# 236088/reflect-sampling-nerf

Hardware: AMD Instinct MI355X
Metric: rays/sec (train step) at 4096 rays x 128 samples, 1/2/4/8 MI355X; PSNR vs ref (higher is better)
Workload: dtype f32

## Files before the change

### reflect_sampling_nerf_amd/csrc/rsn_common.h

```cpp
#pragma once
#include <hip/hip_runtime.h>
#include <stdint.h>
#include <stdio.h>

#include "rsn.h"

#define RSN_K_ENC_PAD 104
#define RSN_K_SH_PAD 40
#define RSN_ENC_ITS (RSN_K_ENC_PAD / 8)
#define RSN_SH_ITS (RSN_K_SH_PAD / 8)
#define RSN_ENC_K16 7
#define RSN_SH_K16 3
#define RSN_AUX_ITS 6

void rsn_set_error(const char* fmt, ...);
int rsn_device_cus();

#define RSN_REQUIRE(cond, code, ...)        \
  do {                                      \
    if (!(cond)) {                          \
      rsn_set_error(__VA_ARGS__);           \
      return (code);                        \
    }                                       \
  } while (0)

#define RSN_TRY(call)                       \
  do {                                      \
    const int rc_ = (call);                 \
    if (rc_ != RSN_OK) return rc_;          \
  } while (0)

#define RSN_HIP(call)                                                                   \
  do {                                                                                  \
    hipError_t e_ = (call);                                                             \
    if (e_ != hipSuccess) {                                                             \
      rsn_set_error("%s failed: %s (%s:%d)", #call, hipGetErrorString(e_), __FILE__, __LINE__); \
      return RSN_ERR_HIP;                                                               \
    }                                                                                   \
  } while (0)

struct RsnPackedLayout {
  int nb;
  int nbm;
  size_t w_x[RSN_MAX_TRUNK_LAYERS];
  size_t w_enc0;
  size_t w_enc_skip;
  size_t b[RSN_MAX_TRUNK_LAYERS];
  size_t w_bh, b_bh;
  size_t w_mid_sh, w_mid_x, b_mid;
  size_t w_rgb, b_rgb;
  size_t wT_x[RSN_MAX_TRUNK_LAYERS];
  size_t wT_enc0, wT_enc_skip;
  size_t wT_bh;
  size_t wT_mid_x;
  size_t wT_rgb;
  size_t v_density;
  size_t h_x[RSN_MAX_TRUNK_LAYERS];
  size_t h_enc0, h_enc_skip, h_bh, h_mid_sh, h_mid_x, h_rgb;
  size_t hT_x[RSN_MAX_TRUNK_LAYERS];
  size_t hT_enc0, hT_enc_skip, hT_bh, hT_mid_x, hT_rgb;
  size_t hT_seed;
  size_t q_stream;
  int q_groups;
  int t_g_begin, t_g_trunk, t_g_encskip, t_g_enc0, t_g_end;
  int q_pf;
  size_t fold_wc, fold_bc, w_fold, b_fold, wT_fold;
  size_t total;
};
#define RSN_RING_GROUP_FRAGS 16
#define RSN_RING_MAX_LAYERS 10
inline bool rsn_ring_training(const rsn_field_desc* d) {
  return (d->mma_mode == RSN_MMA_BF16 || d->mma_mode == RSN_MMA_BF16X6) && d->width == 256 &&
         d->num_layers <= RSN_RING_MAX_LAYERS;
}

int rsn_compute_layout(const rsn_field_desc* desc, RsnPackedLayout* L);

__device__ __forceinline__ float rsn_seed_product(float w, float wd) { return w * wd; }
```

### reflect_sampling_nerf_amd/csrc/rsn_field_bwd.hip

```cpp
#include "rsn_mfma.h"

#include "rsn_field_common.h"
#include "rsn_field_bwd_common.h"

template <int NB, int MMA>
__global__ __launch_bounds__(256) void rsn_field_bwd_kernel(const BwdJobs J) {
  constexpr bool FOLD = MMA == RSN_MMA_F32_FOLDED;
  constexpr int MODE = FOLD ? 0 : MMA;
  constexpr int HIT = FOLD ? 16 : NB * 4;
  constexpr int XITS = (NB * 4 > 16) ? NB * 4 : 16;
  constexpr int WAVE_F4 = (XITS + RSN_AUX_ITS) * 64;
  constexpr int W = NB * 32;
  constexpr bool SBF = MODE == 3;
  __shared__ float4 smem[4 * WAVE_F4];

  const int lane = threadIdx.x & 63;
  const int wid = __builtin_amdgcn_readfirstlane(threadIdx.x >> 6);
  float4* X = smem + wid * WAVE_F4 + lane;
  float* Xf = reinterpret_cast<float*>(X);

  const BwdShared& P = J.s;
  const TileJobs T = tile_space<128>(J);
  const float* __restrict__ pk = P.packed;
  const float4 zero4 = make_float4(0.0f, 0.0f, 0.0f, 0.0f);

  for (long long gtile = blockIdx.x; gtile < T.n_tiles; gtile += gridDim.x) {
    const TileAt ta = tile_at(T, gtile);
    const BwdJob& a = J.j[ta.job];
    const long long n_points = ta.n_points, tile = ta.tile;
    const long long p0 = tile * 128 + wid * 32;
    if (p0 >= n_points) continue;
    int ln = lane;
    asm volatile("" : "+v"(ln));
    const int m = ln & 31, h = ln >> 5;
    const long long p = p0 + m;
    const bool valid = p < n_points;
    const long long pc = valid ? p : n_points - 1;
    const int rows = (int)(n_points - p0 < 32 ? n_points - p0 : 32);
    constexpr bool LOOPST = MODE == 0;
    auto rb_epi = [&](float* base, long long elem, int row_elems) {
      return rowbuf<SBF>(LOOPST ? nullptr : base, elem, rows, row_elems, m, h);
    };
    auto rb_loop = [&](float* base, long long elem, int row_elems) {
      return rowbuf<false>(LOOPST ? base : nullptr, elem, rows, row_elems, m, h);
    };
    const float live = valid ? 1.0f : 0.0f;

    auto bits_at = [&](int l) -> const unsigned* {
      return a.saved.relu_bits + ((((long long)l * (a.act_stride / W)) + pc) * 2 + h) * (NB / 2 > 2 ? NB / 2 : 2);
    };
    HeadGradIn hg;
    head_grad_inputs(a, pc, live, h == 1 && valid, hg);

    X[0] = (h == 1) ? make_float4(hg.dz[0], hg.dz[1], hg.dz[2], 0.0f) : zero4;
    X[64] = zero4; X[128] = zero4; X[192] = zero4;
    {
      const ReluBits<4> mb = load_relu_bits<4>(bits_at(P.num_layers));
      __builtin_amdgcn_sched_barrier(0);
      f32x16 acc[4];
      zero_acc<4>(acc);
      gemm_mode<MODE, 4, 4, true>(acc, pk + P.L.wT_rgb, pk + P.L.hT_rgb, X, 4, ln);
      store_masked_bits<4, SBF>(acc, X, mb, h, rb_epi(a.gout.da_mid, p0 * 128, 128));
    }
    if constexpr (!FOLD) {
      f32x16 acc[NB];
      zero_acc<NB>(acc);
      gemm_mode<MODE, NB, NB, true>(acc, pk + P.L.wT_mid_x, pk + P.L.hT_mid_x, X, 16, ln, rb_loop(a.gout.da_mid, p0 * 128, 128));
      store_act<NB, NB, false, SBF>(acc, X, rb_epi(a.gout.d_bott, p0 * W, W), h);
    }
    {
      const float4 q0 = head_grad_row<false>(h == 0 ? 0 : 1, a, P.density_bias, pc, live, hg);
      const float4 q1 = head_grad_row<false>(h == 0 ? 2 : 3, a, P.density_bias, pc, live, hg);
      X[(HIT + 0) * 64] = q0;
      X[(HIT + 1) * 64] = q1;
      X[(HIT + 2) * 64] = zero4;
      X[(HIT + 3) * 64] = zero4;
      if (valid && a.gout.dz_heads) {
        *reinterpret_cast<float4*>(a.gout.dz_heads + pc * 16 + 4 * h) = q0;
        *reinterpret_cast<float4*>(a.gout.dz_heads + pc * 16 + 8 + 4 * h) = q1;
      }
      const int l = P.num_layers - 1;
      const ReluBits<NB> mb = load_relu_bits<NB>(bits_at(l));
      __builtin_amdgcn_sched_barrier(0);
      f32x16 acc[NB];
      zero_acc<NB>(acc);
      if constexpr (FOLD)
        gemm_mode<MODE, NB, NB, true>(acc, pk + P.L.wT_fold, pk + P.L.hT_bh, X, 16 + 4, ln, rb_loop(a.gout.da_mid, p0 * 128, 128));
      else
        gemm_mode<MODE, NB, NB, true>(acc, pk + P.L.wT_bh, pk + P.L.hT_bh, X, NB * 4 + 4, ln, rb_loop(a.gout.d_bott, p0 * W, W));
      store_masked_bits<NB, SBF>(acc, X, mb, h, rb_epi(a.gout.dy, (long long)l * a.act_stride + p0 * W, W));
    }
    f32x16 eacc[4];
    zero_acc<4>(eacc);
#pragma unroll 1
    for (int l = P.num_layers - 1; l >= 1; --l) {
      if (a.need_input_grad && l == P.skip_layer)
        gemm_mode<MODE, 4, 4, true>(eacc, pk + P.L.wT_enc_skip, pk + P.L.hT_enc_skip, X, NB * 4, ln);
      const ReluBits<NB> mb = load_relu_bits<NB>(bits_at(l - 1));
      __builtin_amdgcn_sched_barrier(0);
      f32x16 acc[NB];
      zero_acc<NB>(acc);
      gemm_mode<MODE, NB, NB, true>(acc, pk + P.L.wT_x[l], pk + P.L.hT_x[l], X, NB * 4, ln,
                          rb_loop(a.gout.dy, (long long)l * a.act_stride + p0 * W, W));
      store_masked_bits<NB, SBF>(acc, X, mb, h, rb_epi(a.gout.dy, (long long)(l - 1) * a.act_stride + p0 * W, W));
    }
    if (LOOPST && !a.need_input_grad) {
      const RowBuf r0 = rb_loop(a.gout.dy, p0 * W, W);
#pragma unroll 4
      for (int it = 0; it < NB * 4; ++it) sv_put_it(r0, it, X[it * 64]);
    }
    if (a.need_input_grad) {
      gemm_mode<MODE, 4, 4, true>(eacc, pk + P.L.wT_enc0, pk + P.L.hT_enc0, X, NB * 4, ln, rb_loop(a.gout.dy, p0 * W, W));
      store_act<4, 4, false>(eacc, X);
      const float* encp = a.saved.enc + pc * RSN_K_ENC_PAD;
      float dvar[3];
#pragma unroll 1
      for (int c = 0; c < 3; ++c) {
        float part = 0.0f;
#pragma unroll 2
        for (int jj = 0; jj < 8; ++jj) {
          const float f = h ? P.freqs[8 + jj] : P.freqs[jj];
          const int u = c * 8 + jj, u2 = u + 24;
          const float gs = Xf[(u >> 2) * 256 + (u & 3)], gc = Xf[(u2 >> 2) * 256 + (u2 & 3)];
          const float fs = encp[(u >> 2) * 8 + 4 * h + (u & 3)], fc = encp[(u2 >> 2) * 8 + 4 * h + (u2 & 3)];
          part += (-0.5f * (f * f)) * (gs * fs + gc * fc);
        }
        const float tot = part + __shfl_xor(part, 32, 64);
        if (c == 0) dvar[0] = tot; else if (c == 1) dvar[1] = tot; else dvar[2] = tot;
      }
      if (h == 0 && valid && a.gout.d_input) a.gout.d_input[pc] = input_grad_of_dvar(a, pc, dvar);
    }
  }
}

static int launch_bwd_jobs(const rsn_field_desc* d, const float* packed, BwdJob* js, int n, void* stream) {
  RSN_REQUIRE(n >= 1 && n <= RSN_MAX_JOBS, RSN_ERR_INVALID_ARGUMENT, "n_jobs=%d (1..%d)", n, RSN_MAX_JOBS);
  BwdJobs J = {};
  RSN_TRY(rsn_fill_shared(J.s, d, packed));
  for (int k = 0; k < n; ++k) {
    BwdJob& a = js[k];
    RSN_REQUIRE(a.saved.relu_bits && a.saved.heads && a.gout.dy, RSN_ERR_INVALID_ARGUMENT,
                "job %d: saved relu_bits / heads and gout.dy are required", k);
    RSN_REQUIRE(!a.need_input_grad || (a.saved.enc && a.gout.d_input), RSN_ERR_INVALID_ARGUMENT,
                "job %d: need_input_grad needs saved.enc and gout.d_input", k);
    RSN_REQUIRE(a.mode == RSN_MODE_INF || (a.fwd.raw_density && a.fwd.diff && a.fwd.tint), RSN_ERR_INVALID_ARGUMENT,
                "job %d: forward values raw_density/diff/tint are required", k);
    RSN_REQUIRE(!(a.gin.ray_pn_loss || a.gin.ray_ori_loss) || (a.mode == RSN_MODE_FRUSTUM && a.gin.weights),
                RSN_ERR_INVALID_ARGUMENT, "job %d: fused normal losses need the level's weights (frustum levels only)", k);
    RSN_REQUIRE(!a.gin.ray_pn_loss || (a.saved.normals && a.fwd.pred_normals), RSN_ERR_INVALID_ARGUMENT,
                "job %d: ray_pn_loss needs saved.normals and the forward pred_normals", k);
    RSN_REQUIRE(!a.gin.ray_ori_loss || a.fwd.n_dot_d, RSN_ERR_INVALID_ARGUMENT, "job %d: ray_ori_loss needs the forward n_dot_d", k);
    if (a.n_rays <= 0) continue;
    a.act_stride = (long long)a.n_rays * a.S * (long long)d->width;
    J.j[J.n_jobs++] = a;
  }
  if (J.n_jobs == 0) return RSN_OK;
  const long long n_tiles = rsn_job_tiles(J, 128);
  const int cached_cus = rsn_device_cus();
  const long long grid = n_tiles < (long long)cached_cus ? n_tiles : (long long)cached_cus;
  hipStream_t st = (hipStream_t)stream;
  const bool x6 = d->mma_mode == RSN_MMA_BF16X6;
  if (rsn_ring_training(d))
    return x6 ? rsn_launch_field_x6_bwd(n_tiles, st, J) : rsn_launch_field_bf16_bwd(rsn_job_tiles(J, 256), st, J);
#define RSN_LAUNCH_BWD(NBV)                                                                                  \
  do {                                                                                                       \
    if (x6) hipLaunchKernelGGL((rsn_field_bwd_kernel<NBV, 1>), dim3((unsigned)grid), dim3(256), 0, st, J);    \
    else if (d->mma_mode == RSN_MMA_BF16)   \
      hipLaunchKernelGGL((rsn_field_bwd_kernel<NBV, 3>), dim3((unsigned)grid), dim3(256), 0, st, J);              \
    else if (d->mma_mode == RSN_MMA_F32_FOLDED)             \
      hipLaunchKernelGGL((rsn_field_bwd_kernel<NBV, 4>), dim3((unsigned)grid), dim3(256), 0, st, J);        \
    else hipLaunchKernelGGL((rsn_field_bwd_kernel<NBV, 0>), dim3((unsigned)grid), dim3(256), 0, st, J);       \
  } while (0)
  switch (d->width) {
    case 256: RSN_LAUNCH_BWD(8); break;
    case 128: RSN_LAUNCH_BWD(4); break;
    case 64: RSN_LAUNCH_BWD(2); break;
    default: RSN_REQUIRE(false, RSN_ERR_UNSUPPORTED, "width=%d unsupported", d->width);
  }
#undef RSN_LAUNCH_BWD
  RSN_HIP(hipGetLastError());
  return RSN_OK;
}

static int launch_bwd(const rsn_field_desc* d, const float* pk, BwdJob& a, void* st) { return launch_bwd_jobs(d, pk, &a, 1, st); }

extern "C" int rsn_field_backward_jobs(const rsn_field_desc* desc, const float* packed, int32_t n_jobs,
                                       const rsn_field_bwd_job* jobs, void* stream) {
// ... 52 lines not shown
```

### reflect_sampling_nerf_amd/csrc/rsn_mfma.h

```cpp
#pragma once
#include "rsn_common.h"

typedef float f32x16 __attribute__((ext_vector_type(16)));

#define RSN_MODE_FRUSTUM 0
#define RSN_MODE_INF 1
#define RSN_MODE_GAUSS 2
#define RSN_MODE_EMB 3

__device__ __forceinline__ float softplus_f(float x) { return x > 20.0f ? x : log1pf(expf(x)); }
__device__ __forceinline__ float sigmoid_f(float x) { return 1.0f / (1.0f + expf(-x)); }

__device__ __forceinline__ float sincos_big(float a, int quad) {
  const float q = rintf(a * 0.63661977236758134308f);
  float r = __builtin_fmaf(-q, 1.5707963705062866f, a);
  r = __builtin_fmaf(-q, -4.371138828673793e-08f, r);
  r = __builtin_fmaf(-q, -1.7151245100058819e-15f, r);
  const int n = (int)q + quad;
  const float s = r * r;
  const float ps = r + r * s * (-1.6666654611e-1f + s * (8.3321608736e-3f + s * (-1.9515295891e-4f)));
  const float pc =
      1.0f + s * (-0.5f + s * (4.166664568298827e-2f + s * (-1.388731625493765e-3f + s * 2.443315711809948e-5f)));
  const float v = (n & 1) ? pc : ps;
  return (n & 2) ? -v : v;
// ... 571 lines not shown
    f32x16 c = acc[nb0 + t];
    c = __builtin_amdgcn_mfma_f32_32x32x16_bf16(s3, b, c, 0, 0, 0);
    c = __builtin_amdgcn_mfma_f32_32x32x16_bf16(s2, b, c, 0, 0, 0);
    c = __builtin_amdgcn_mfma_f32_32x32x16_bf16(s1, b, c, 0, 0, 0);
    acc[nb0 + t] = c;
  }
}

template <int NBO>
__device__ __forceinline__ void gemm_f32_bits(f32x16 (&acc)[NBO], const float* __restrict__ w32seg, const float* __restrict__ wd,
                                              const ReluBits<NBO>& m, int lane) {
  static_assert(NBO % 2 == 0, "two fragment buffers of NBO / 2 blocks");
  constexpr int NH = NBO / 2, NK = 2 * NBO;
  const WBuf wp = wbuf_make(w32seg, lane);
  const float* __restrict__ wdl = wd + 4 * (lane >> 5);
  float4 fa[NH][2], fb[NH][2];
  load_w32_pair<NBO, NH>(fa, wp, 0, 0);
  const SeedWords mw = seed_words<NBO>(m);
  float4 dlo = *reinterpret_cast<const float4*>(wdl), dhi = *reinterpret_cast<const float4*>(wdl + 8);
#pragma unroll 1
  for (int kk = 0; kk < NK; ++kk) {
    load_w32_pair<NBO, NH>(fb, wp, kk, NH);
    const int kn = (kk + 1 < NK) ? kk + 1 : kk;
    const float4 nlo = *reinterpret_cast<const float4*>(wdl + 16 * kn), nhi = *reinterpret_cast<const float4*>(wdl + 16 * kn + 8);
    const bf16x8 bc = bits_bf16x8(mw, kk);
    mma16_bits_f32<NBO, NH>(acc, fa, dlo, dhi, bc, 0);
    __builtin_amdgcn_sched_barrier(0);
    load_w32_pair<NBO, NH>(fa, wp, kn, 0);
    mma16_bits_f32<NBO, NH>(acc, fb, dlo, dhi, bc, NH);
    __builtin_amdgcn_sched_barrier(0);
    dlo = nlo; dhi = nhi;
  }
}

typedef float f32x4 __attribute__((ext_vector_type(4)));

template <int NBO>
__device__ __forceinline__ void zero_acc16(f32x4 (&acc)[NBO][2][2]) {
#pragma unroll
  for (int nb = 0; nb < NBO; ++nb)
#pragma unroll
    for (int q = 0; q < 4; ++q) acc[nb][q >> 1][q & 1] = f32x4{0.0f, 0.0f, 0.0f, 0.0f};
}

struct Lane16 {
  int ol;
  int kh;
};
__device__ __forceinline__ Lane16 lane16(int lane) {
  Lane16 g;
  g.ol = (lane & 15) + 2 * (lane & 16);
  g.kh = lane >> 5;
  return g;
}

__device__ __forceinline__ bf16x8 piece(const BSplit& b, int k) { return k == 0 ? b.s1 : (k == 1 ? b.s2 : b.s3); }
constexpr int x9_wp(int p) { constexpr int t[9] = {2, 2, 1, 2, 1, 0, 1, 0, 0}; return t[p]; }
constexpr int x9_bp(int p) { constexpr int t[9] = {2, 1, 2, 0, 1, 2, 0, 1, 0}; return t[p]; }
template <int NBO, int NQ>
__device__ __forceinline__ void mma16s(f32x4 (&acc)[NBO][2][2], const bf16x8 (&w)[NQ][2][3], const BSplit (&b)[2], int nb0) {
#pragma unroll
  for (int t = 0; t < NQ; ++t)
#pragma unroll
    for (int p = 0; p < 9; ++p)
#pragma unroll
      for (int q = 0; q < 4; ++q)
        acc[nb0 + t][q >> 1][q & 1] = __builtin_amdgcn_mfma_f32_16x16x32_bf16(w[t][q >> 1][x9_wp(p)], piece(b[q & 1], x9_bp(p)),
                                                                              acc[nb0 + t][q >> 1][q & 1], 0, 0, 0);
}

template <int NQ>
__device__ __forceinline__ void load_w16s(bf16x8 (&w)[NQ][2][3], const WBuf& wp, int s, int nbo, int nb0) {
#pragma unroll
  for (int t = 0; t < NQ; ++t)
#pragma unroll
    for (int rh = 0; rh < 2; ++rh)
#pragma unroll
      for (int sp = 0; sp < 3; ++sp) {
        const u32x4 v = __builtin_amdgcn_raw_buffer_load_b128(wp.r, wp.voff + rh * 256u, (unsigned)(((2 * s * nbo + nb0 + t) * 3 + sp) * 1024), 0);
        w[t][rh][sp] = __builtin_bit_cast(bf16x8, v);
      }
}

template <int NBO>
__device__ __forceinline__ void gemm_bf16_s16(f32x4 (&acc)[NBO][2][2], const float* __restrict__ wseg, const float4* xl, int n_k32,
                                              int lane) {
  static_assert(NBO % 2 == 0, "an even number of fragment buffers' worth of blocks");
  constexpr int NQ = NBO >= 4 ? NBO / 4 : 1, NC = NBO / NQ;
  const Lane16 g = lane16(lane);
  WBuf wp = wbuf_make(wseg, lane);
  wp.voff = (unsigned)g.ol * 16u + (unsigned)g.kh * (NBO * 3072u);
  const float4* xb = xl - lane + g.ol + g.kh * 128;
  bf16x8 wa[NQ][2][3], wb[NQ][2][3];
  load_w16s<NQ>(wa, wp, 0, NBO, 0);
  BSplit bc[2] = {split8<3>(xb[0], xb[64]), split8<3>(xb[16], xb[80])};
  const int s1 = n_k32 > 1 ? 1 : 0;
  float4 x0lo = xb[4 * s1 * 64], x0hi = xb[(4 * s1 + 1) * 64], x1lo = xb[4 * s1 * 64 + 16], x1hi = xb[(4 * s1 + 1) * 64 + 16];
#pragma unroll 1
  for (int s = 0; s < n_k32; ++s) {
    const int sn = (s + 1 < n_k32) ? s + 1 : s;
    const int s2 = (s + 2 < n_k32) ? s + 2 : sn;
    BSplit bn[2];
#pragma unroll
    for (int c = 0; c < NC; ++c) {
      if (c & 1) load_w16s<NQ>(wa, wp, c + 1 < NC ? s : sn, NBO, c + 1 < NC ? (c + 1) * NQ : 0);
      else load_w16s<NQ>(wb, wp, s, NBO, (c + 1) * NQ);
      __builtin_amdgcn_sched_barrier(0);
      if (c == 0) bn[0] = split8<3>(x0lo, x0hi);
      if (c == 1) bn[1] = split8<3>(x1lo, x1hi);
      if (c == NC - 1) {
        x0lo = xb[4 * s2 * 64]; x0hi = xb[(4 * s2 + 1) * 64];
        x1lo = xb[4 * s2 * 64 + 16]; x1hi = xb[(4 * s2 + 1) * 64 + 16];
      }
      if (c & 1) mma16s<NBO, NQ>(acc, wb, bc, c * NQ); else mma16s<NBO, NQ>(acc, wa, bc, c * NQ);
#pragma unroll
      for (int m = 0; m < NQ * 36; ++m) {
        __builtin_amdgcn_sched_group_barrier(0x008, 1, 0);
        if (c < 2) __builtin_amdgcn_sched_group_barrier(0x002, 2, 0);
      }
      if (c == NC - 1) __builtin_amdgcn_sched_group_barrier(0x100, 4, 0);
      __builtin_amdgcn_sched_barrier(0);
    }
    bc[0] = bn[0];
    bc[1] = bn[1];
  }
}

template <int NQ>
__device__ __forceinline__ void load_w32s(float4 (&f)[NQ][2][2], const WBuf& b, int s, int nbo, int nb0) {
#pragma unroll
  for (int t = 0; t < NQ; ++t)
#pragma unroll
    for (int rh = 0; rh < 2; ++rh)
#pragma unroll
      for (int j = 0; j < 2; ++j) {
        const u32x4 v = __builtin_amdgcn_raw_buffer_load_b128(b.r, b.voff + rh * 256u, (unsigned)(((4 * s + j) * nbo + nb0 + t) * 1024), 0);
        f[t][rh][j] = make_float4(__uint_as_float(v.x), __uint_as_float(v.y), __uint_as_float(v.z), __uint_as_float(v.w));
      }
}

template <int NBO>
__device__ __forceinline__ void gemm_f32_x9_s16(f32x4 (&acc)[NBO][2][2], const float* __restrict__ w32seg, const float4* xl,
                                                int n_k32, int lane) {
  static_assert(NBO % 2 == 0, "an even number of fragment buffers' worth of blocks");
  constexpr int NQ = NBO >= 4 ? NBO / 4 : 1, NC = NBO / NQ, UQ = 2 * NQ, NU = 2 * NBO;
  const Lane16 g = lane16(lane);
  WBuf wp = wbuf_make(w32seg, lane);
  wp.voff = (unsigned)g.ol * 16u + (unsigned)g.kh * (NBO * 2048u);
  const float4* xb = xl - lane + g.ol + g.kh * 128;
  float4 fa[NQ][2][2], fb[NQ][2][2];
  load_w32s<NQ>(fa, wp, 0, NBO, 0);
  load_w32s<NQ>(fb, wp, 0, NBO, NQ);
  BSplit bc[2] = {split8<3>(xb[0], xb[64]), split8<3>(xb[16], xb[80])};
  const int s1 = n_k32 > 1 ? 1 : 0;
  float4 x0lo = xb[4 * s1 * 64], x0hi = xb[(4 * s1 + 1) * 64], x1lo = xb[4 * s1 * 64 + 16], x1hi = xb[(4 * s1 + 1) * 64 + 16];
  BSplit w = split8<3>(fa[0][0][0], fa[0][0][1]);
  BSplit bn[2] = {bc[0], bc[1]};
#pragma unroll 1
  for (int s = 0; s < n_k32; ++s) {
    const int sn = (s + 1 < n_k32) ? s + 1 : s;
    const int s2 = (s + 2 < n_k32) ? s + 2 : sn;
#pragma unroll
    for (int u = 0; u < NU; ++u) {
      const int un = (u + 1) % NU, cn = (un / UQ) & 1, tn = (un / 2) % NQ;
      const BSplit wn = cn ? split8<3>(fb[tn][un & 1][0], fb[tn][un & 1][1]) : split8<3>(fa[tn][un & 1][0], fa[tn][un & 1][1]);
      const bool reload = u % UQ == UQ - 1;
      if (reload) {
        const int c = u / UQ, c2 = (c + 2) % NC;
        if (c & 1) load_w32s<NQ>(fb, wp, c + 2 < NC ? s : sn, NBO, c2 * NQ);
        else load_w32s<NQ>(fa, wp, c + 2 < NC ? s : sn, NBO, c2 * NQ);
      }
      if (u == NU - 2) bn[0] = split8<3>(x0lo, x0hi);
      if (u == NU - 1) {
        bn[1] = split8<3>(x1lo, x1hi);
        x0lo = xb[4 * s2 * 64]; x0hi = xb[(4 * s2 + 1) * 64];
        x1lo = xb[4 * s2 * 64 + 16]; x1hi = xb[(4 * s2 + 1) * 64 + 16];
      }
#pragma unroll
      for (int p = 0; p < 9; ++p)
#pragma unroll
        for (int ph = 0; ph < 2; ++ph)
          acc[u >> 1][u & 1][ph] = __builtin_amdgcn_mfma_f32_16x16x32_bf16(piece(w, x9_wp(p)), piece(bc[ph], x9_bp(p)),
                                                                           acc[u >> 1][u & 1][ph], 0, 0, 0);
#pragma unroll
      for (int m = 0; m < 18; ++m) {
        __builtin_amdgcn_sched_group_barrier(0x008, 1, 0);
        if (reload && m < NQ * 4) __builtin_amdgcn_sched_group_barrier(0x020, 1, 0);
        if (u >= NU - 2) __builtin_amdgcn_sched_group_barrier(0x002, 6, 0);
        else __builtin_amdgcn_sched_group_barrier(0x002, 3, 0);
      }
      if (u == NU - 1) __builtin_amdgcn_sched_group_barrier(0x100, 4, 0);
      __builtin_amdgcn_sched_barrier(0);
      w = wn;
    }
    bc[0] = bn[0];
    bc[1] = bn[1];
  }
}

__device__ __forceinline__ unsigned bit_mask(int word, int pos) {
  unsigned m;
// ... 181 lines not shown
```

### reflect_sampling_nerf_amd/csrc/rsn_pack.hip

```cpp
#include <stdarg.h>
#include <stdlib.h>
#include <string.h>

#include <string>
#include <vector>

#include "rsn_common.h"

static thread_local std::string g_last_error;

void rsn_set_error(const char* fmt, ...) {
  char buf[1024];
  va_list ap;
  va_start(ap, fmt);
  vsnprintf(buf, sizeof(buf), fmt, ap);
  va_end(ap);
  g_last_error = buf;
}

extern "C" const char* rsn_last_error(void) { return g_last_error.c_str(); }

int rsn_device_cus() {
  static int cache[64] = {0};
  int dev = 0;
// ... 29 lines not shown
  size_t off = 0;
  const size_t x_seg = (size_t)(L->nb * 4) * L->nb * blk;
  const size_t enc_seg = (size_t)RSN_ENC_ITS * L->nb * blk;
  for (int l = 0; l < d->num_layers; ++l) {
    if (l == 0) {
      L->w_enc0 = off;
      off += enc_seg;
    } else {
      L->w_x[l] = off;
      off += x_seg;
      if (l == d->skip_layer) {
        L->w_enc_skip = off;
        off += enc_seg;
      }
    }
    L->b[l] = off;
    off += (size_t)d->width;
  }
  L->w_bh = off;
  off += (size_t)(L->nb * 4) * (L->nb + 1) * blk;
  L->b_bh = off;
  off += (size_t)(L->nb + 1) * 32;
  L->w_mid_sh = off;
  off += (size_t)RSN_SH_ITS * L->nbm * blk;
  L->w_mid_x = off;
  off += (size_t)(L->nb * 4) * L->nbm * blk;
  L->b_mid = off;
  off += (size_t)d->mid_width;
  L->w_rgb = off;
  off += (size_t)(L->nbm * 4) * 1 * blk;
  L->b_rgb = off;
  off += 32;
  for (int l = 1; l < d->num_layers; ++l) {
    L->wT_x[l] = off;
    off += x_seg;
  }
  const size_t encT_seg = (size_t)(L->nb * 4) * 4 * blk;
  L->wT_enc0 = off;
  off += encT_seg;
  L->wT_enc_skip = off;
  off += (d->skip_layer >= 1) ? encT_seg : 0;
  L->wT_bh = off;
  off += (size_t)(L->nb * 4 + 4) * L->nb * blk;
  L->wT_mid_x = off;
  off += (size_t)(L->nbm * 4) * L->nb * blk;
  L->wT_rgb = off;
  off += (size_t)4 * L->nbm * blk;
  L->v_density = off;
  off += (size_t)d->width;
  const size_t hx_seg = (size_t)(L->nb * 2) * L->nb * 3 * blk;
  const size_t henc_seg = (size_t)RSN_ENC_K16 * L->nb * 3 * blk;
  L->h_enc0 = off;
  off += henc_seg;
  for (int l = 1; l < d->num_layers; ++l) {
    L->h_x[l] = off;
    off += hx_seg;
  }
  L->h_enc_skip = off;
  off += (d->skip_layer >= 1) ? henc_seg : 0;
  L->h_bh = off;
  off += (size_t)(L->nb * 2) * (L->nb + 1) * 3 * blk;
  L->h_mid_sh = off;
  off += (size_t)RSN_SH_K16 * L->nbm * 3 * blk;
  L->h_mid_x = off;
  off += (size_t)(L->nb * 2) * L->nbm * 3 * blk;
  L->h_rgb = off;
  off += (size_t)(L->nbm * 2) * 1 * 3 * blk;
  for (int l = 1; l < d->num_layers; ++l) {
    L->hT_x[l] = off;
    off += hx_seg;
  }
  const size_t hencT_seg = (size_t)(L->nb * 2) * 4 * 3 * blk;
  L->hT_enc0 = off;
  off += hencT_seg;
  L->hT_enc_skip = off;
  off += (d->skip_layer >= 1) ? hencT_seg : 0;
  L->hT_bh = off;
  off += (size_t)(L->nb * 2 + 2) * L->nb * 3 * blk;
  L->hT_mid_x = off;
  off += (size_t)(L->nbm * 2) * L->nb * 3 * blk;
  L->hT_rgb = off;
  off += (size_t)2 * L->nbm * 3 * blk;
  L->hT_seed = (d->mma_mode == RSN_MMA_F32_FOLDED && d->num_layers >= 2) ? L->hT_x[d->num_layers - 1] : 0;
  L->q_pf = 1;
  if ((d->mma_mode == RSN_MMA_BF16 || d->mma_mode == RSN_MMA_BF16X6) && d->width == 256) {
    const int pf = d->mma_mode == RSN_MMA_BF16X6 ? 3 : 1;
    L->q_pf = pf;
    L->q_groups = pf * ((64 * (d->skip_layer >= 1 ? 2 : 1) + (d->num_layers - 1) * 128 + 16 + 128 + 16 + 64 + 16) / 16);
    L->q_stream = off;
    off += (size_t)L->q_groups * 16 * blk;
    int tg = L->q_groups;
    L->t_g_begin = tg;
    tg += pf * (1 + 4 + 9);
    L->t_g_trunk = tg;
    L->t_g_encskip = -1;
    for (int l = d->num_layers - 1; l >= 1; --l) {
      if (l == d->skip_layer) { L->t_g_encskip = tg; tg += pf * 4; }
      tg += pf * 8;
    }
    L->t_g_enc0 = tg;
    tg += pf * 4;
    L->t_g_end = tg;
    off += (size_t)(tg - L->q_groups) * 16 * blk;
  }
  if (d->mma_mode == RSN_MMA_F32_FOLDED) {
    const size_t pw = (size_t)(d->param_width > 0 ? d->param_width : d->width);
    L->fold_wc = off;
    off += ((size_t)d->mid_width * pw + 3) / 4 * 4;
    L->fold_bc = off;
    off += (size_t)d->mid_width;
    L->w_fold = off;
    off += (size_t)(L->nb * 4) * (L->nbm + 1) * blk;
    L->b_fold = off;
    off += (size_t)(L->nbm + 1) * 32;
    L->wT_fold = off;
    off += (size_t)(L->nbm * 4 + 4) * L->nb * blk;
  }
  L->total = off;
  return RSN_OK;
}

namespace {
int enc_column(int u, int f0, int nf) {
  if (u < 3 * nf) return (u / nf) * 16 + f0 + u % nf;
  if (u < 6 * nf) return 48 + ((u - 3 * nf) / nf) * 16 + f0 + u % nf;
  return (u < 6 * nf + 3 && f0 == 0) ? 96 + (u - 6 * nf) : -1;
}
int sh_column(int u, int first, int n) { return (u < n && first + u < RSN_SH_DIM) ? first + u : -1; }

int enc_slot_to_column(int k) { return enc_column((k >> 3) * 4 + (k & 3), 8 * ((k >> 2) & 1), 8); }
int sh_slot_to_column(int k) { return sh_column((k >> 3) * 4 + (k & 3), 17 * ((k >> 2) & 1), 17); }
int enc16_slot_to_column(int k) { return enc_column((k >> 5) * 8 + (k & 7), 4 * ((k >> 3) & 3), 4); }
int sh16_slot_to_column(int k) { return sh_column((k >> 5) * 8 + (k & 7), 9 * ((k >> 3) & 3), 9); }

int perm16_row_to_feature(int n) {
  const int b = n >> 4, g = (n >> 2) & 3, r = n & 3;
  return 32 * (b >> 1) + 8 * g + 4 * (b & 1) + r;
}

struct HeadRows { int head, row0, n_rows; };
constexpr HeadRows kHeads[5] = {{0, 0, 1}, {1, 1, 3}, {2, 4, 3}, {3, 8, 1}, {4, 12, 3}};
}

extern "C" int rsn_train_saved_layout(const rsn_field_desc* d, int32_t* enc_cols, int32_t* sh_cols, int32_t* narrow_bf16,
                                      int32_t* enc_map, int32_t* sh_map) {
  RSN_REQUIRE(d && enc_cols && sh_cols && narrow_bf16 && enc_map && sh_map, RSN_ERR_INVALID_ARGUMENT, "a pointer is NULL");
  RsnPackedLayout L;
  const int rc = rsn_compute_layout(d, &L);
  if (rc != RSN_OK) return rc;
  const bool ring = rsn_ring_training(d);
  *enc_cols = ring ? 128 : RSN_K_ENC_PAD; *sh_cols = ring ? 64 : RSN_K_SH_PAD;
  *narrow_bf16 = (ring && d->mma_mode == RSN_MMA_BF16) ? 1 : 0;
  for (int s = 0; s < 128; ++s) enc_map[s] = ring ? enc16_slot_to_column(s) : enc_slot_to_column(s);
  for (int s = 0; s < 64; ++s) sh_map[s] = ring ? sh16_slot_to_column(s) : sh_slot_to_column(s);
  return RSN_OK;
}

extern "C" size_t rsn_packed_weights_bytes(const rsn_field_desc* desc) {
  RsnPackedLayout L;
  if (rsn_compute_layout(desc, &L) != RSN_OK) return 0;
  return L.total * sizeof(float);
}

#define PACK_MAX_ROWS 288
#define PACK_MAX_COLS 256
#define PACK_MAX_SRC 6
// ... 265 lines not shown
  j = gemm(p->bottleneck_w, W, L.wT_bh, NB * 4, NB, 1);
  rows_natural(*j, W); cols_natural(*j, W, 0);
  j = gemm(nullptr, 0, L.wT_bh + (size_t)(NB * 4) * NB * 256, 4, NB, 3);
  heads_src(*j, 0, heads_w, W); rows_natural(*j, W); cols_headsT(*j, false);
  j = gemm(p->mid_w, mid_in, L.wT_mid_x, NBM * 4, NB, 1);
  rows_natural(*j, W, RSN_SH_DIM); cols_natural(*j, MW, 0);
  j = gemm(p->rgb_w, MW, L.wT_rgb, 4, NBM, 1);
  rows_natural(*j, MW);
  for (int c = 0; c < 3; ++c) j->col[4 + c] = (int16_t)c;
  rows_natural(*bias(p->density_w, L.v_density, WP), W);

  if (L.q_stream != 0) {
    int frag = 0;
    auto ring = [&](const float* w, int ld, int ks, int nbo16, int transpose = 0) {
      PackJob* q = gemm(w, ld, L.q_stream + (size_t)frag * 256 * L.q_pf, ks, nbo16, transpose);
      q->layout = L.q_pf == 3 ? 2 : 1;
      frag += ks * nbo16;
      return q;
    };
    for (int l = 0; l < n_layers; ++l) {
      if (l >= 1) {
        j = ring(p->trunk_w[l], in_f(l), 8, 16);
        rows_perm16(*j, WP, W); cols_natural(*j, W, x_off(l));
      }
      if (l == 0 || l == skip) {
        j = ring(p->trunk_w[l], in_f(l), 4, 16);
        rows_perm16(*j, WP, W); cols_slots(*j, 128, enc16_slot_to_column);
      }
    }
    j = ring(nullptr, W, 8, 2);
    heads_src(*j, 1, heads_w, W); heads_rows(*j, 0); cols_natural(*j, W, 0);
    j = ring(p->bottleneck_w, W, 8, 16);
    rows_perm16(*j, WP, W); cols_natural(*j, W, 0);
    j = ring(p->mid_w, mid_in, 2, 8);
    rows_perm16(*j, MW, MW); cols_slots(*j, 64, sh16_slot_to_column);
    j = ring(p->mid_w, mid_in, 8, 8);
    rows_perm16(*j, MW, MW); cols_natural(*j, W, RSN_SH_DIM);
    j = ring(p->rgb_w, MW, 4, 4);
    rows_rgb(*j); cols_natural(*j, MW, 0);
    RSN_REQUIRE(frag * L.q_pf == L.q_groups * 16, RSN_ERR_INVALID_ARGUMENT, "16x32 stream: %d fragments, layout says %d groups",
                frag, L.q_groups);
    j = ring(p->rgb_w, MW, 2, 8, 1);
    rows_perm16(*j, MW, MW);
    for (int c = 0; c < 3; ++c) j->col[8 + c] = (int16_t)c;
    j = ring(p->mid_w, mid_in, 4, 16, 1);
    rows_perm16(*j, WP, W, RSN_SH_DIM); cols_natural(*j, MW, 0);
    j = ring(p->bottleneck_w, W, 8, 16, 1);
    rows_perm16(*j, WP, W); cols_natural(*j, W, 0);
    j = ring(nullptr, 0, 1, 16, 3);
    heads_src(*j, 0, heads_w, W); rows_perm16(*j, WP, W); cols_headsT(*j, true);
    for (int l = n_layers - 1; l >= 0; --l) {
      if (l == 0 || l == skip) {
        j = ring(p->trunk_w[l], in_f(l), 8, 8, 1);
        rows_from(*j, 128, [](int n) { return enc16_slot_to_column(perm16_row_to_feature(n)); }); cols_natural(*j, W, 0);
      }
      if (l >= 1) {
        j = ring(p->trunk_w[l], in_f(l), 8, 16, 1);
        rows_perm16(*j, WP, W, x_off(l)); cols_natural(*j, W, 0);
      }
    }
    RSN_REQUIRE(frag * L.q_pf == L.t_g_end * 16, RSN_ERR_INVALID_ARGUMENT, "transposed 16x32 stream: %d fragments, layout says %d groups",
                frag, L.t_g_end);
  }

  if (d->mma_mode == RSN_MMA_F32_FOLDED) {
    const float* wc = packed + L.fold_wc;
    j = gemm(wc, W, L.w_fold, NB * 4, NBM + 1);
    heads_src(*j, 1, heads_w, W); rows_natural(*j, MW); heads_rows(*j, MW); cols_natural(*j, W, 0);
    j = bias(packed + L.fold_bc, L.b_fold, MW + 32);
    heads_src(*j, 1, heads_b, 0); rows_natural(*j, MW); heads_rows(*j, MW);
    j = gemm(wc, W, L.wT_fold, NBM * 4, NB, 1);
    rows_natural(*j, W); cols_natural(*j, MW, 0);
    j = gemm(nullptr, 0, L.wT_fold + (size_t)(NBM * 4) * NB * 256, 4, NB, 3);
    heads_src(*j, 0, heads_w, W); rows_natural(*j, W); cols_headsT(*j, false);
  }

  auto split = [&](size_t src, int n_it, int nbo, size_t dst, size_t kscale = 0) {
    splits.push_back(SplitSeg{(unsigned)src, (unsigned)dst, (short)n_it, (short)nbo, 0, (unsigned)kscale});
  };
  if (d->mma_mode == RSN_MMA_F32 || d->mma_mode == RSN_MMA_F32_FOLDED) {
    if (L.hT_seed != 0) split(L.wT_x[n_layers - 1], NB * 4, NB, L.hT_seed, L.v_density);
    if (d->mma_mode == RSN_MMA_F32_FOLDED) {
      for (int l = 1; l + 1 < n_layers; ++l) split(L.wT_x[l], NB * 4, NB, L.hT_x[l]);
      if (skip >= 1) split(L.wT_enc_skip, NB * 4, 4, L.hT_enc_skip);
      split(L.wT_enc0, NB * 4, 4, L.hT_enc0);
    }
    return RSN_OK;
  }
  split(L.w_enc0, RSN_ENC_ITS, NB, L.h_enc0);
  for (int l = 1; l < n_layers; ++l) {
    split(L.w_x[l], NB * 4, NB, L.h_x[l]);
    split(L.wT_x[l], NB * 4, NB, L.hT_x[l]);
  }
  if (skip >= 1) {
    split(L.w_enc_skip, RSN_ENC_ITS, NB, L.h_enc_skip);
    split(L.wT_enc_skip, NB * 4, 4, L.hT_enc_skip);
  }
  split(L.wT_enc0, NB * 4, 4, L.hT_enc0);
  split(L.w_bh, NB * 4, NB + 1, L.h_bh);
  split(L.wT_bh, NB * 4 + 4, NB, L.hT_bh);
  split(L.w_mid_sh, RSN_SH_ITS, NBM, L.h_mid_sh);
  split(L.w_mid_x, NB * 4, NBM, L.h_mid_x);
  split(L.wT_mid_x, NBM * 4, NB, L.hT_mid_x);
  split(L.w_rgb, NBM * 4, 1, L.h_rgb);
  split(L.wT_rgb, 4, NBM, L.hT_rgb);
  return RSN_OK;
}

thread_local std::vector<PackJob> t_jobs;
thread_local std::vector<SplitSeg> t_splits;

int validate_and_build(const rsn_field_desc* d, const rsn_field_params* p, float* packed, size_t packed_bytes) {
  RsnPackedLayout L;
  const int rc = rsn_compute_layout(d, &L);
  if (rc != RSN_OK) return rc;
  RSN_REQUIRE(p != nullptr && packed != nullptr, RSN_ERR_INVALID_ARGUMENT, "params/packed is NULL");
  RSN_REQUIRE(packed_bytes >= L.total * sizeof(float), RSN_ERR_WORKSPACE,
              "packed buffer too small: %zu < %zu bytes", packed_bytes, L.total * sizeof(float));
  t_jobs.clear(); t_splits.clear();
  return build_jobs(d, p, packed, L, t_jobs, t_splits);
}

}

static int launch_fold(const rsn_field_desc* d, const rsn_field_params* p, float* packed, hipStream_t st) {
  if (d->mma_mode != RSN_MMA_F32_FOLDED) return RSN_OK;
  RsnPackedLayout L;
  RSN_TRY(rsn_compute_layout(d, &L));
  const int w = d->param_width > 0 ? d->param_width : d->width, n = d->mid_width * w + d->mid_width;
  hipLaunchKernelGGL(rsn_fold_kernel, dim3((unsigned)((n + 255) / 256)), dim3(256), 0, st, p->mid_w, p->mid_b, p->bottleneck_w,
                     p->bottleneck_b, w, d->mid_width, packed + L.fold_wc, packed + L.fold_bc);
  RSN_HIP(hipGetLastError());
  return RSN_OK;
}

extern "C" int rsn_pack_weights(const rsn_field_desc* d, const rsn_field_params* p, float* packed,
                                size_t packed_bytes, void* stream) {
  const int rc = validate_and_build(d, p, packed, packed_bytes);
  if (rc != RSN_OK) return rc;
  hipStream_t st = (hipStream_t)stream;
  RSN_TRY(launch_fold(d, p, packed, st));
  for (const PackJob& j : t_jobs) {
    hipLaunchKernelGGL(rsn_pack_kernel, dim3((unsigned)job_blocks(j)), dim3(256), 0, st, j);
    RSN_HIP(hipGetLastError());
  }
  for (const SplitSeg& s : t_splits) {
    hipLaunchKernelGGL(rsn_pack_split_kernel, dim3((unsigned)split_blocks(s)), dim3(256), 0, st, packed + s.src, (int)s.n_it,
                       (int)s.nbo, packed + s.dst, s.kscale ? packed + s.kscale : nullptr);
    RSN_HIP(hipGetLastError());
  }
  return RSN_OK;
}

extern "C" size_t rsn_pack_table_bytes(void) { return sizeof(PackTable); }

extern "C" int rsn_pack_weights_table(const rsn_field_desc* d, const rsn_field_params* p, float* packed,
                                      size_t packed_bytes, void* table, size_t table_bytes, int32_t rebuild_table,
                                      void* stream) {
  RSN_REQUIRE(table != nullptr && table_bytes >= sizeof(PackTable), RSN_ERR_WORKSPACE,
              "job table buffer too small: %zu < %zu bytes", table_bytes, sizeof(PackTable));
  const int rc = validate_and_build(d, p, packed, packed_bytes);
  if (rc != RSN_OK) return rc;
  RSN_REQUIRE((int)t_jobs.size() <= PACK_MAX_JOBS && (int)t_splits.size() <= SPLIT_MAX_SEGS, RSN_ERR_UNSUPPORTED,
              "%zu pack jobs / %zu split segments exceed the table", t_jobs.size(), t_splits.size());
  hipStream_t st = (hipStream_t)stream;
  static thread_local PackTable host_table;
// ... 30 lines not shown
```

Before: 93150.

## Use split-bf16 16x16 MFMA path for folded-mode backward trunk layers

In the folded f32 mode, the backward trunk loop now runs on the bf16x3-split 16x16x32 MFMA GEMM instead of the generic f32 gemm_mode path, with per-16-row relu masks and a fused store of the incoming gradient rows. A separate split copy of the last trunk layer's transposed weights (hT_last, reusing the hT_bh slot) is packed because hT_x for that layer already holds the density-seeded weights. The aim is to replace slower f32 MFMA work with split-bf16 MFMA while keeping near-f32 accuracy. It adds packing work, alters the store pattern and relies on the hT_bh region being large enough for the reused slot.

```diff
diff --git a/reflect_sampling_nerf_amd/csrc/rsn_common.h b/reflect_sampling_nerf_amd/csrc/rsn_common.h
--- a/reflect_sampling_nerf_amd/csrc/rsn_common.h
+++ b/reflect_sampling_nerf_amd/csrc/rsn_common.h
@@ -1,5 +1,6 @@
 #pragma once
 #include <hip/hip_runtime.h>
+#include <stddef.h>
 #include <stdint.h>
 #include <stdio.h>
 
@@ -64,9 +65,13 @@
   int q_groups;
   int t_g_begin, t_g_trunk, t_g_encskip, t_g_enc0, t_g_end;
   int q_pf;
+  unsigned hT_last;
   size_t fold_wc, fold_bc, w_fold, b_fold, wT_fold;
   size_t total;
 };
+static_assert(offsetof(RsnPackedLayout, fold_wc) == offsetof(RsnPackedLayout, hT_last) + 4 &&
+                  offsetof(RsnPackedLayout, hT_last) == offsetof(RsnPackedLayout, q_pf) + 4,
+              "hT_last fills the padding behind q_pf");
 #define RSN_RING_GROUP_FRAGS 16
 #define RSN_RING_MAX_LAYERS 10
 inline bool rsn_ring_training(const rsn_field_desc* d) {
diff --git a/reflect_sampling_nerf_amd/csrc/rsn_field_bwd.hip b/reflect_sampling_nerf_amd/csrc/rsn_field_bwd.hip
--- a/reflect_sampling_nerf_amd/csrc/rsn_field_bwd.hip
+++ b/reflect_sampling_nerf_amd/csrc/rsn_field_bwd.hip
@@ -92,17 +92,34 @@
     }
     f32x16 eacc[4];
     zero_acc<4>(eacc);
+    auto rb16 = [&](float* base, long long elem, int row_elems) {
+      return rowbuf<false>(base, elem, rows, row_elems, ln & 15, (ln >> 4) & 1);
+    };
+    auto bits16_at = [&](int l, int ph) -> const unsigned* {
+      const long long q = p0 + (ln & 15) + 16 * ph, qc = q < n_points ? q : n_points - 1;
+      return a.saved.relu_bits + ((((long long)l * (a.act_stride / W)) + qc) * 2 + ((ln >> 4) & 1)) * (NB / 2 > 2 ? NB / 2 : 2);
+    };
 #pragma unroll 1
     for (int l = P.num_layers - 1; l >= 1; --l) {
       if (a.need_input_grad && l == P.skip_layer)
         gemm_mode<MODE, 4, 4, true>(eacc, pk + P.L.wT_enc_skip, pk + P.L.hT_enc_skip, X, NB * 4, ln);
-      const ReluBits<NB> mb = load_relu_bits<NB>(bits_at(l - 1));
-      __builtin_amdgcn_sched_barrier(0);
-      f32x16 acc[NB];
-      zero_acc<NB>(acc);
-      gemm_mode<MODE, NB, NB, true>(acc, pk + P.L.wT_x[l], pk + P.L.hT_x[l], X, NB * 4, ln,
-                          rb_loop(a.gout.dy, (long long)l * a.act_stride + p0 * W, W));
-      store_masked_bits<NB, SBF>(acc, X, mb, h, rb_epi(a.gout.dy, (long long)(l - 1) * a.act_stride + p0 * W, W));
+      if constexpr (FOLD) {
+        const ReluBits<NB> mb[2] = {load_relu_bits<NB>(bits16_at(l - 1, 0)), load_relu_bits<NB>(bits16_at(l - 1, 1))};
+        __builtin_amdgcn_sched_barrier(0);
+        f32x4 acc[NB][2][2];
+        zero_acc16<NB>(acc);
+        gemm_bf16_s16<NB>(acc, pk + (l == P.num_layers - 1 ? (size_t)P.L.hT_last : P.L.hT_x[l]), X, NB, ln,
+                          rb16(a.gout.dy, (long long)l * a.act_stride + p0 * W, W));
+        store_masked_bits16<NB>(acc, X, mb, ln);
+      } else {
+        const ReluBits<NB> mb = load_relu_bits<NB>(bits_at(l - 1));
+        __builtin_amdgcn_sched_barrier(0);
+        f32x16 acc[NB];
+        zero_acc<NB>(acc);
+        gemm_mode<MODE, NB, NB, true>(acc, pk + P.L.wT_x[l], pk + P.L.hT_x[l], X, NB * 4, ln,
+                            rb_loop(a.gout.dy, (long long)l * a.act_stride + p0 * W, W));
+        store_masked_bits<NB, SBF>(acc, X, mb, h, rb_epi(a.gout.dy, (long long)(l - 1) * a.act_stride + p0 * W, W));
+      }
     }
     if (LOOPST && !a.need_input_grad) {
       const RowBuf r0 = rb_loop(a.gout.dy, p0 * W, W);
diff --git a/reflect_sampling_nerf_amd/csrc/rsn_mfma.h b/reflect_sampling_nerf_amd/csrc/rsn_mfma.h
--- a/reflect_sampling_nerf_amd/csrc/rsn_mfma.h
+++ b/reflect_sampling_nerf_amd/csrc/rsn_mfma.h
@@ -677,9 +677,20 @@
       }
 }
 
-template <int NBO>
+__device__ __forceinline__ void sv_put16(const float*, int, int, bool, const float4, const float4) {}
+__device__ __forceinline__ void sv_put16(const RowBuf& b, int it, int ph, bool live, const float4 lo, const float4 hi) {
+  const unsigned at = b.voff + (unsigned)ph * 16u * b.lim + (unsigned)it * 32u;
+  const unsigned o0 = (live && (unsigned)it * 32u < b.lim) ? at : 0x80000000u;
+  const unsigned o1 = (live && (unsigned)it * 32u + 32u < b.lim) ? at + 32u : 0x80000000u;
+  const u32x4 v0 = {__float_as_uint(lo.x), __float_as_uint(lo.y), __float_as_uint(lo.z), __float_as_uint(lo.w)};
+  const u32x4 v1 = {__float_as_uint(hi.x), __float_as_uint(hi.y), __float_as_uint(hi.z), __float_as_uint(hi.w)};
+  __builtin_amdgcn_raw_buffer_store_b128(v0, b.r, o0, 0, RSN_SAVED_ROW_AUX);
+  __builtin_amdgcn_raw_buffer_store_b128(v1, b.r, o1, 0, RSN_SAVED_ROW_AUX);
+}
+
+template <int NBO, class SV = const float*>
 __device__ __forceinline__ void gemm_bf16_s16(f32x4 (&acc)[NBO][2][2], const float* __restrict__ wseg, const float4* xl, int n_k32,
-                                              int lane) {
+                                              int lane, SV save = nullptr) {
   static_assert(NBO % 2 == 0, "an even number of fragment buffers' worth of blocks");
   constexpr int NQ = NBO >= 4 ? NBO / 4 : 1, NC = NBO / NQ;
   const Lane16 g = lane16(lane);
@@ -688,7 +699,17 @@
   const float4* xb = xl - lane + g.ol + g.kh * 128;
   bf16x8 wa[NQ][2][3], wb[NQ][2][3];
   load_w16s<NQ>(wa, wp, 0, NBO, 0);
-  BSplit bc[2] = {split8<3>(xb[0], xb[64]), split8<3>(xb[16], xb[80])};
+  BSplit bc[2];
+  if (sv_on(save)) {
+    const float4 p0lo = xb[0], p0hi = xb[64], p1lo = xb[16], p1hi = xb[80];
+    bc[0] = split8<3>(p0lo, p0hi);
+    bc[1] = split8<3>(p1lo, p1hi);
+    sv_put16(save, 2 * g.kh, 0, true, p0lo, p0hi);
+    sv_put16(save, 2 * g.kh, 1, true, p1lo, p1hi);
+  } else {
+    bc[0] = split8<3>(xb[0], xb[64]);
+    bc[1] = split8<3>(xb[16], xb[80]);
+  }
   const int s1 = n_k32 > 1 ? 1 : 0;
   float4 x0lo = xb[4 * s1 * 64], x0hi = xb[(4 * s1 + 1) * 64], x1lo = xb[4 * s1 * 64 + 16], x1hi = xb[(4 * s1 + 1) * 64 + 16];
 #pragma unroll 1
@@ -703,6 +724,8 @@
       __builtin_amdgcn_sched_barrier(0);
       if (c == 0) bn[0] = split8<3>(x0lo, x0hi);
       if (c == 1) bn[1] = split8<3>(x1lo, x1hi);
+      if (c == 0 && sv_on(save)) sv_put16(save, 4 * sn + 2 * g.kh, 0, s + 1 < n_k32, x0lo, x0hi);
+      if (c == 1 && sv_on(save)) sv_put16(save, 4 * sn + 2 * g.kh, 1, s + 1 < n_k32, x1lo, x1hi);
       if (c == NC - 1) {
         x0lo = xb[4 * s2 * 64]; x0hi = xb[(4 * s2 + 1) * 64];
         x1lo = xb[4 * s2 * 64 + 16]; x1hi = xb[(4 * s2 + 1) * 64 + 16];
@@ -712,6 +735,7 @@
       for (int m = 0; m < NQ * 36; ++m) {
         __builtin_amdgcn_sched_group_barrier(0x008, 1, 0);
         if (c < 2) __builtin_amdgcn_sched_group_barrier(0x002, 2, 0);
+        if (c < 2 && sv_on(save) && (m == 8 || m == 20)) __builtin_amdgcn_sched_group_barrier(0x040, 1, 0);
       }
       if (c == NC - 1) __builtin_amdgcn_sched_group_barrier(0x100, 4, 0);
       __builtin_amdgcn_sched_barrier(0);
diff --git a/reflect_sampling_nerf_amd/csrc/rsn_pack.hip b/reflect_sampling_nerf_amd/csrc/rsn_pack.hip
--- a/reflect_sampling_nerf_amd/csrc/rsn_pack.hip
+++ b/reflect_sampling_nerf_amd/csrc/rsn_pack.hip
@@ -135,6 +135,7 @@
   L->hT_rgb = off;
   off += (size_t)2 * L->nbm * 3 * blk;
   L->hT_seed = (d->mma_mode == RSN_MMA_F32_FOLDED && d->num_layers >= 2) ? L->hT_x[d->num_layers - 1] : 0;
+  L->hT_last = (d->mma_mode == RSN_MMA_F32_FOLDED && d->num_layers >= 2) ? (unsigned)L->hT_bh : 0u;
   L->q_pf = 1;
   if ((d->mma_mode == RSN_MMA_BF16 || d->mma_mode == RSN_MMA_BF16X6) && d->width == 256) {
     const int pf = d->mma_mode == RSN_MMA_BF16X6 ? 3 : 1;
@@ -566,6 +567,7 @@
     if (L.hT_seed != 0) split(L.wT_x[n_layers - 1], NB * 4, NB, L.hT_seed, L.v_density);
     if (d->mma_mode == RSN_MMA_F32_FOLDED) {
       for (int l = 1; l + 1 < n_layers; ++l) split(L.wT_x[l], NB * 4, NB, L.hT_x[l]);
+      if (L.hT_last != 0) split(L.wT_x[n_layers - 1], NB * 4, NB, L.hT_last);
       if (skip >= 1) split(L.wT_enc_skip, NB * 4, 4, L.hT_enc_skip);
       split(L.wT_enc0, NB * 4, 4, L.hT_enc0);
     }
```

Result: faster. 94780 (median of 6 runs) (+1.7%).
